# lh3/miniasm

Hardware: AMD Instinct MI355X
Metric: PAF overlaps processed/sec (hit-filter->trans-reduce->GFA) (higher is better)
Workload: dtype u32

## Files before the change

miniasm_amd/csrc/hits.hip:

```cpp
#include "mahip_internal.hpp"

#define COL_QID 0
#define COL_QS 1
#define COL_QE 2
#define COL_TN 3
#define COL_TS 4
#define COL_TE 5
#define COL_ML 6
#define COL_BL 7
#define DEAD 0x80000000u

__global__ __launch_bounds__(256) void k_hit_keys(const ma_hit_t *__restrict__ h, size_t n, uint64_t *__restrict__ key,
                                                   uint32_t *__restrict__ val, uint32_t *__restrict__ keep, unsigned long long *__restrict__ ctr,
                                                   uint32_t q_beg, uint32_t q_end, int bi, int full)
{
	uint32_t cnt = 0;
	for (size_t i = (size_t)blockIdx.x * 256 + threadIdx.x; i < n; i += (size_t)gridDim.x * 256) {
		uint64_t k = h[i].qns;
		uint32_t q = (uint32_t)(k >> 32);
		int in = q >= q_beg && q < q_end;
		cnt += in;
		if (full) key[i] = k, val[i] = (uint32_t)i;
		else key[i] = (uint64_t)q << bi | i;
		if (keep) keep[i] = in;
// ... 244 lines not shown
		else if (i0 < n) q0 = (uint32_t)(skey[i0] >> bi);
		if (q0 > n_seq) q0 = n_seq;
		if (q1 > n_seq) q1 = n_seq;
		uint32_t qprev = __shfl_up(q1, 1, 64);
		if ((threadIdx.x & 63) == 0 && i0 && i0 <= n) qprev = (uint32_t)(skey[i0 - 1] >> bi);
		if (i0 <= n) {
			const uint32_t lo = i0 ? qprev + 1 : q_lo, hi = q0 < q_hi ? q0 : q_hi;
			for (uint32_t r = lo > q_lo ? lo : q_lo; r <= hi; ++r) goff[r] = (uint32_t)i0;
		}
		if (i0 + 1 <= n) { const uint32_t hi = q1 < q_hi ? q1 : q_hi; for (uint32_t r = q0 + 1 > q_lo ? q0 + 1 : q_lo; r <= hi; ++r) goff[r] = (uint32_t)(i0 + 1); }
	}
}

#define SUB_BLOCKS (2u * MA_STREAM_BLOCKS)
static uint32_t sub_chunk(uint32_t R) { uint64_t waves = 4ull * grid_for(R, 4, SUB_BLOCKS), k = waves ? R / waves : 1; return (uint32_t)(k < 1 ? 1 : k > 16 ? 16 : k); }
#define EV_PAD 0xffffffffu
#define SUB_REG_MAX_HITS 512u
#define SUB_CHUNK 16u
#define SUB_LDS_EVENTS 8192u


struct SubFuse {
	const uint2 *cut_sub;
	int min_span, max_hang, min_ovlp;
	uint8_t *r_live;
};
struct SubAcc { uint32_t n_cut, n_flt; uint64_t dp; };

__device__ __forceinline__ uint32_t sub_len(uint2 s) { return s.y - (s.x & 0x7fffffffu); }
__device__ __forceinline__ bool subs_live(uint2 rq, uint2 rt) { return !(rq.x & DEAD) && !(rt.x & DEAD); }

__device__ __forceinline__ int hit_cut(uint2 rq, uint2 rt, uint32_t &qs, uint32_t &qe, uint32_t &ts, uint32_t &te, uint32_t ml, int min_span)
{
	return subs_live(rq, rt) && mc_cut(&qs, &qe, &ts, &te, ml >> 31, (int32_t)rq.x, rq.y, (int32_t)rt.x, rt.y, min_span);
}
__device__ __forceinline__ void store_cut_cols(const HitCols &c, size_t i, uint32_t qs, uint32_t qe, uint32_t ts, uint32_t te, uint32_t oqs, uint32_t oqe, uint32_t ots, uint32_t ote)
{
	if (qs != oqs) c.qs[i] = qs;
	if (qe != oqe) c.qe[i] = qe;
	if (ts != ots) c.ts[i] = ts;
	if (te != ote) c.te[i] = te;
}
__device__ __forceinline__ int hit_flt(uint32_t q, uint32_t qs, uint32_t qe, uint32_t tn, uint32_t ts, uint32_t te, uint32_t ml, uint2 sq, uint2 st,
                                       int max_hang, int min_ovlp, uint64_t &dp, uint8_t *r_live)
{
	mc_arc_t a;
	const uint32_t ql = sub_len(sq), tl = sub_len(st);
	const int r = mc_hit2arc(q, qs, qe, tn, ts, te, ml >> 31, (int)ql, (int)tl, max_hang, .5f, min_ovlp, &a);
	if (r >= 0 || r == MC_HT_QCONT || r == MC_HT_TCONT) {
		dp += r >= 0 ? (uint32_t)r : r == MC_HT_QCONT ? ql : tl;
		r_live[q] = 1;
		return 1;
	}
	return 0;
}
__device__ __forceinline__ void hit_contained_flags(uint32_t q, uint32_t qs, uint32_t qe, uint32_t t, uint32_t ts, uint32_t te, uint32_t ml, uint2 sq, uint2 st,
                                                    int max_hang, float int_frac, int min_ovlp, uint8_t *r_cont, uint8_t *r_used)
{
	mc_arc_t a;
	const int r = mc_hit2arc(q, qs, qe, t, ts, te, ml >> 31, (int)sub_len(sq), (int)sub_len(st), max_hang, int_frac, min_ovlp, &a);
	if (r == MC_HT_QCONT) r_cont[q] = 1;
	else if (r == MC_HT_TCONT) r_cont[t] = 1;
	r_used[q] = 1; r_used[t] = 1;
}

__device__ __forceinline__ int fuse_cut_flt_v(const HitCols &c, uint32_t i, const SubFuse &f, uint32_t q, uint2 rq, uint32_t tn,
                                              uint32_t &qs, uint32_t &qe, uint32_t ml, uint32_t bl, SubAcc &acc, uint2 rt, uint32_t ts, uint32_t te)
{
	int keep = 0;
	const uint32_t oqs = qs, oqe = qe, ots = ts, ote = te;
	if (hit_cut(rq, rt, qs, qe, ts, te, ml, f.min_span)) {
		++acc.n_cut;
		if (hit_flt(q, qs, qe, tn, ts, te, ml, rq, rt, f.max_hang, f.min_ovlp, acc.dp, f.r_live)) {
			keep = 1; ++acc.n_flt;
			store_cut_cols(c, i, qs, qe, ts, te, oqs, oqe, ots, ote);
		}
	}
	if (!keep) c.bl[i] = bl | DEAD;
	return keep;
}
__device__ __forceinline__ int fuse_cut_flt(const HitCols &c, uint32_t i, const SubFuse &f, uint32_t q, uint2 rq, uint32_t tn,
                                            uint32_t &qs, uint32_t &qe, uint32_t ml, uint32_t bl, SubAcc &acc)
{
	return fuse_cut_flt_v(c, i, f, q, rq, tn, qs, qe, ml, bl, acc, f.cut_sub[tn], c.ts[i], c.te[i]);
}

struct SubPre { uint32_t beg, end; uint32_t bl[2], ml[2], qs[2], qe[2], tn[2], ts[2], te[2]; uint2 rt[2], rq; };

template <bool FUSE>
__device__ __forceinline__ void sub_preload(const HitCols &c, const uint32_t *__restrict__ goff, uint32_t q, unsigned lane, SubPre &p)
{
	p.beg = goff[q]; p.end = goff[q + 1];
	const uint32_t H = p.end - p.beg;
#pragma unroll
	for (int h = 0; h < 2; ++h) {
		const uint32_t i = p.beg + h * 64 + lane;
		p.bl[h] = DEAD; p.ml[h] = p.qs[h] = p.qe[h] = p.tn[h] = p.ts[h] = p.te[h] = 0;
		if (H <= 128u && i < p.end) {
			p.bl[h] = c.bl[i]; p.ml[h] = c.ml[i]; p.qs[h] = c.qs[i]; p.qe[h] = c.qe[i]; p.tn[h] = c.tn[i];
			if (FUSE) { p.ts[h] = c.ts[i]; p.te[h] = c.te[i]; }
		}
	}
}

struct SubGather { const uint32_t *pos; uint32_t pstride, pmask; const ma_hit_t *aos; uint32_t *sidx; uint32_t n, chunk, q_lo; };
struct GBounds { uint32_t beg, end; };
struct GKeys { uint32_t beg, end, j[2]; };
struct GRecs { uint32_t beg, end, j[2]; uint4 a[2], b[2]; };

__device__ __forceinline__ uint32_t gather_pos(const SubGather &g, size_t i)
{
	return g.pos[i * g.pstride] & g.pmask;
}
__device__ __forceinline__ void gather_bounds(const uint32_t *__restrict__ goff, uint64_t q, uint32_t n_seq, GBounds &b)
{
	const uint32_t qc = q < n_seq ? (uint32_t)q : n_seq - 1;
	b.beg = goff[qc]; b.end = goff[qc + 1];
}
__device__ __forceinline__ void gather_keys(const SubGather &g, const GBounds &b, unsigned lane, GKeys &k)
{
	k.beg = b.beg; k.end = b.end;
#pragma unroll
	for (int h = 0; h < 2; ++h) {
		const uint32_t i = b.beg + h * 64 + lane, ic = i < g.n ? i : g.n - 1;
		k.j[h] = g.pos[(size_t)ic * g.pstride];
	}
}
__device__ __forceinline__ void gather_recs(const SubGather &g, const GKeys &k, unsigned lane, GRecs &r)
{
	r.beg = k.beg; r.end = k.end;
	const bool mine = k.end - k.beg <= 128u;
	const uint32_t mask = g.pmask;
#pragma unroll
	for (int h = 0; h < 2; ++h) {
		const uint32_t i = k.beg + h * 64 + lane;
		r.j[h] = (mine && i < k.end) ? (k.j[h] & mask) : 0u;
		const uint4 *p = (const uint4*)(g.aos + r.j[h]);
		r.a[h] = p[0]; r.b[h] = p[1];
	}
}
template <int GATHER>
__device__ __forceinline__ void gather_store(const HitCols &c, const SubGather &g, uint32_t i, uint32_t j, uint4 a, uint4 b)
{
	c.qid[i] = a.y; c.qs[i] = a.x; c.qe[i] = a.z; c.tn[i] = a.w;
	c.ts[i] = b.x; c.te[i] = b.y; c.ml[i] = b.z; c.bl[i] = b.w & ~DEAD;
	if (GATHER == 1) g.sidx[i] = j;
}

template <int ITEMS, bool FUSE, int GATHER = 0>
__device__ __forceinline__ uint32_t sub_group_regs(const HitCols &c, uint32_t q, uint32_t beg, uint32_t end, int min_dp, float min_iden,
                                                   int end_clip, uint2 *__restrict__ sub, unsigned lane, const SubFuse &f, SubAcc &acc, const SubPre *pre = nullptr,
                                                   const SubGather *g = nullptr)
{
	uint32_t x[ITEMS];
	int live_any = 0, ev_any = 0;
	uint2 rq = make_uint2(0, 0);
	if (FUSE) rq = pre ? pre->rq : f.cut_sub[q];
	if (GATHER && !pre) {
		constexpr int HB = 4;
#pragma unroll
		for (int h0 = 0; h0 < ITEMS / 2; h0 += HB) {
			uint32_t jj[HB];
			uint4 aa[HB], bb[HB];
#pragma unroll
			for (int k = 0; k < HB; ++k) { const uint32_t i = beg + (h0 + k) * 64 + lane; jj[k] = (h0 + k < ITEMS / 2 && i < end) ? gather_pos(*g, i) : 0u; }
#pragma unroll
			for (int k = 0; k < HB; ++k) { const uint4 *p = (const uint4*)(g->aos + jj[k]); aa[k] = p[0]; bb[k] = p[1]; }
#pragma unroll
			for (int k = 0; k < HB; ++k) {
				const int h = h0 + k;
				const uint32_t i = beg + h * 64 + lane;
				if (h < ITEMS / 2) {
					x[2 * h] = x[2 * h + 1] = EV_PAD;
					if (i < end) {
						uint32_t es, ee;
						gather_store<GATHER>(c, *g, i, jj[k], aa[k], bb[k]);
						live_any = 1;
						if (mc_sub_ok(q, aa[k].x, aa[k].z, aa[k].w, (int32_t)(bb[k].z & 0x7fffffffu), (int32_t)(bb[k].w & ~DEAD), min_iden, end_clip, &es, &ee)) x[2 * h] = es, x[2 * h + 1] = ee, ev_any = 1;
					}
				}
			}
		}
	} else
#pragma unroll
	for (int h = 0; h < ITEMS / 2; ++h) {
		uint32_t i = beg + h * 64 + lane;
		x[2 * h] = x[2 * h + 1] = EV_PAD;
		if (i < end) {
			uint32_t bl, ml, qs, qe, tn, es, ee;
			int alive;
			if (pre) {
				bl = pre->bl[h]; ml = pre->ml[h]; qs = pre->qs[h]; qe = pre->qe[h]; tn = pre->tn[h];
				alive = !(bl & DEAD) && (!FUSE || fuse_cut_flt_v(c, i, f, q, rq, tn, qs, qe, ml, bl, acc, pre->rt[h], pre->ts[h], pre->te[h]));
			} else {
				bl = c.bl[i]; ml = c.ml[i]; qs = c.qs[i]; qe = c.qe[i]; tn = c.tn[i];
				alive = !(bl & DEAD) && (!FUSE || fuse_cut_flt(c, i, f, q, rq, tn, qs, qe, ml, bl, acc));
			}
			if (alive) {
				live_any = 1;
				if (mc_sub_ok(q, qs, qe, tn, (int32_t)(ml & 0x7fffffffu), (int32_t)bl, min_iden, end_clip, &es, &ee)) x[2 * h] = es, x[2 * h + 1] = ee, ev_any = 1;
			}
		}
	}
	if (wv_ballot(live_any) == 0) { if (lane == 0) sub[q] = make_uint2(0, 0); return 0; }
	if (wv_ballot(ev_any) == 0) { if (lane == 0) sub[q] = make_uint2(DEAD, 0); return 0; }
	wave_sort_regs<ITEMS>(x, lane);
	int net = 0;
#pragma unroll
	for (int r = 0; r < ITEMS; ++r) if (x[r] != EV_PAD) net += (x[r] & 1) ? -1 : 1;
	int dp = wv_scan_incl_i32(net, lane) - net;
	const uint32_t NONE = 0xffffffffu;
	uint32_t cur_up = NONE, last_up = NONE, pend_pos = NONE, pend_idx = 0, best_s = 0;
	uint64_t best = 0;
#pragma unroll
	for (int r = 0; r < ITEMS; ++r) {
		uint32_t e = x[r];
		if (e == EV_PAD) continue;
		int old = dp;
		dp += (e & 1) ? -1 : 1;
		if (old < min_dp && dp >= min_dp) cur_up = last_up = e >> 1;
		else if (old >= min_dp && dp < min_dp) {
			if (cur_up != NONE) {
				uint64_t cand = (uint64_t)((e >> 1) - cur_up) << 32 | (0xffffffffu - (lane * ITEMS + r));
				if (cand > best) best = cand, best_s = cur_up;
				cur_up = NONE;
			} else pend_pos = e >> 1, pend_idx = lane * ITEMS + r;
		}
	}
	const uint32_t carry = wv_scan_last_u32(last_up, NONE, lane);
	const uint32_t before = wv_prev_lane_u32(carry, NONE, lane);
	if (pend_pos != NONE && before != NONE) {
		uint64_t cand = (uint64_t)(pend_pos - before) << 32 | (0xffffffffu - pend_idx);
		if (cand > best) best = cand, best_s = before;
	}
	uint64_t gbest = wv_max_u64_full(best);
	uint32_t len = (uint32_t)(gbest >> 32);
	if (len == 0) { if (lane == 0) sub[q] = make_uint2(DEAD, 0); return 0; }
	uint64_t own = wv_ballot(best == gbest);
	uint32_t s = wv_read_lane_u32(best_s, __ffsll((long long)own) - 1);
	if (lane == 0) sub[q] = make_uint2((s - (uint32_t)end_clip) & 0x7fffffffu, s + len + (uint32_t)end_clip);
	return 1;
}

__device__ __forceinline__ unsigned sub_block_id()
{
	const unsigned b = blockIdx.x, g8 = gridDim.x & ~7u;
	return b < g8 ? (b & 7u) * (g8 >> 3) + (b >> 3) : b;
}
#if defined(__HIP__) && defined(__clang__)
#define SUB_WPE_ATTR(F, C, G) __attribute__((amdgpu_waves_per_eu(sub_wpe(F, C, G))))
#else
#define SUB_WPE_ATTR(F, C, G)
#endif
#ifndef SUB_WPE_G0
#define SUB_WPE_G0 7
#endif
#ifndef SUB_WPE_F0
#define SUB_WPE_F0 6
#endif
constexpr unsigned sub_wpe(bool fuse, int cls, int gather) { return gather && cls == 0 ? SUB_WPE_G0 : fuse && cls == 1 ? 5 : fuse && cls == 0 ? SUB_WPE_F0 : 0; }
template <bool FUSE>
__device__ __forceinline__ void sub_flush_acc(unsigned long long *ctr, const SubAcc &acc)
{
	if (FUSE) { blk_add_u64(&ctr[CT_CUT], acc.n_cut); blk_add_u64(&ctr[CT_LIVE], acc.n_flt); blk_add_u64(&ctr[CT_TOTDP], acc.dp); }
}

template <bool FUSE, int CLS, int GATHER = 0>
__global__ __launch_bounds__(256) SUB_WPE_ATTR(FUSE, CLS, GATHER) void k_hit_sub(HitCols c, const uint32_t *__restrict__ goff, uint32_t n_seq,
                                                  int min_dp, float min_iden, int end_clip, uint2 *__restrict__ sub,
                                                  uint32_t *__restrict__ ovf, unsigned long long *__restrict__ ctr, SubFuse f, SubGather g)
{
	const unsigned lane = threadIdx.x & 63, wave = threadIdx.x >> 6;
	uint32_t n_kept = 0;
	SubAcc acc = {0, 0, 0};
	const uint32_t chunk = g.chunk ? g.chunk : 1u;
	if (CLS == 0 && GATHER) {
		const uint64_t stride = (uint64_t)gridDim.x * 4;
		uint64_t q = (uint64_t)g.q_lo + sub_block_id() * 4 + wave;
		GBounds bn;
		GKeys kn;
		GRecs cur, nxt;
		gather_bounds(goff, q, n_seq, bn); gather_keys(g, bn, lane, kn); gather_recs(g, kn, lane, cur);
		gather_bounds(goff, q + stride, n_seq, bn); gather_keys(g, bn, lane, kn);
		gather_bounds(goff, q + 2 * stride, n_seq, bn);
		while (q < n_seq) {
			const uint32_t beg = cur.beg, end = cur.end, H = end - beg;
#pragma unroll
			for (int h = 0; h < 2; ++h) {
				const uint32_t i = beg + h * 64 + lane;
				gather_store<GATHER>(c, g, (H <= 128u && i < end) ? i : g.n + lane, cur.j[h], cur.a[h], cur.b[h]);
			}
			__builtin_amdgcn_sched_barrier(0);
			gather_recs(g, kn, lane, nxt);
			gather_keys(g, bn, lane, kn);
			gather_bounds(goff, q + 3 * stride, n_seq, bn);
			__builtin_amdgcn_sched_barrier(0);
			if (H == 0) { if (lane == 0) sub[q] = make_uint2(0, 0); }
			else if (H <= 128) {
				SubPre pre;
				pre.beg = beg; pre.end = end;
#pragma unroll
				for (int h = 0; h < 2; ++h) {
					pre.bl[h] = cur.b[h].w & ~DEAD; pre.ml[h] = cur.b[h].z; pre.qs[h] = cur.a[h].x; pre.qe[h] = cur.a[h].z; pre.tn[h] = cur.a[h].w;
					pre.ts[h] = pre.te[h] = 0;
				}
				if (H <= 64) n_kept += sub_group_regs<2, false>(c, (uint32_t)q, beg, end, min_dp, min_iden, end_clip, sub, lane, f, acc, &pre);
				else n_kept += sub_group_regs<4, false>(c, (uint32_t)q, beg, end, min_dp, min_iden, end_clip, sub, lane, f, acc, &pre);
			}
			cur = nxt; q += stride;
		}
	} else
	if (CLS == 0) {
		const uint32_t stride = gridDim.x * 4;
		uint32_t q = g.q_lo + sub_block_id() * 4 + wave;
		SubPre cur, nxt;
		if (q < n_seq) sub_preload<FUSE>(c, goff, q, lane, cur);
		while (q < n_seq) {
			const uint32_t qn = q + stride;
			if (FUSE) {
				cur.rq = f.cut_sub[q];
#pragma unroll
				for (int h = 0; h < 2; ++h) cur.rt[h] = (cur.bl[h] & DEAD) ? make_uint2(DEAD, 0) : f.cut_sub[cur.tn[h]];
			}
			if (qn < n_seq) sub_preload<FUSE>(c, goff, qn, lane, nxt);
			const uint32_t beg = cur.beg, end = cur.end, H = end - beg;
			if (H == 0) { if (lane == 0) sub[q] = make_uint2(0, 0); }
			else if (H <= 64) n_kept += sub_group_regs<2, FUSE>(c, q, beg, end, min_dp, min_iden, end_clip, sub, lane, f, acc, &cur);
			else if (H <= 128) n_kept += sub_group_regs<4, FUSE>(c, q, beg, end, min_dp, min_iden, end_clip, sub, lane, f, acc, &cur);
			cur = nxt; q = qn;
		}
	} else
	for (uint64_t qb = (uint64_t)g.q_lo + (uint64_t)(sub_block_id() * 4 + wave) * chunk; qb < n_seq; qb += (uint64_t)gridDim.x * 4 * chunk) {
	const bool in = lane < chunk && qb + lane < n_seq;
	const uint32_t beg_l = in ? goff[qb + lane] : 0, end_l = in ? goff[qb + lane + 1] : 0, H_l = end_l - beg_l;
	unsigned long long todo = wv_ballot(CLS == 1 ? (H_l > 128 && H_l <= 256) : H_l > 256);
	while (todo) {
		const int qbit = __ffsll((long long)todo) - 1;
		todo &= todo - 1;
		const uint32_t q = (uint32_t)qb + (uint32_t)qbit;
		const uint32_t beg = __shfl(beg_l, qbit, 64), end = __shfl(end_l, qbit, 64), H = end - beg;
		if (CLS == 1) {
			if (H > 128 && H <= 256) n_kept += sub_group_regs<8, FUSE, GATHER>(c, q, beg, end, min_dp, min_iden, end_clip, sub, lane, f, acc, nullptr, &g);
		} else {
			if (H > 256 && H <= SUB_REG_MAX_HITS) n_kept += sub_group_regs<16, FUSE, GATHER>(c, q, beg, end, min_dp, min_iden, end_clip, sub, lane, f, acc, nullptr, &g);
			else if (H > SUB_REG_MAX_HITS) {
				if (GATHER)
					for (uint32_t i = beg + lane; i < end; i += 64) {
						const uint32_t j = gather_pos(g, i);
						const uint4 *p = (const uint4*)(g.aos + j);
						gather_store<GATHER>(c, g, i, j, p[0], p[1]);
					}
				if (lane == 0) { unsigned long long k = atomicAdd(&ctr[CT_OVF], 1ull); ovf[k] = q; }
			}
		}
	}
	}
	blk_add_u64(&ctr[CT_REMAIN], lane == 0 ? n_kept : 0);
	sub_flush_acc<FUSE>(ctr, acc);
}

__device__ __forceinline__ uint64_t sub_sweep(const uint32_t *ev, uint32_t *up, uint32_t nev, int min_dp, unsigned lane)
{
	const uint64_t lt = wv_lt(lane), le = wv_le(lane);
	int carry = 0;
	uint32_t nup = 0, ndown = 0;
	uint64_t best = 0;
	for (uint32_t base = 0; base < nev; base += 64) {
		uint32_t i = base + lane;
		int valid = i < nev;
		uint32_t e = valid ? ev[i] : 0;
		int is_end = e & 1;
		uint64_t ms = wv_ballot(valid && !is_end), me = wv_ballot(valid && is_end);
		int dp = carry + __popcll(ms & le) - __popcll(me & le);
		int old = dp - (is_end ? -1 : 1);
		int isup = valid && old < min_dp && dp >= min_dp;
		int isdn = valid && old >= min_dp && dp < min_dp;
		uint64_t mu = wv_ballot(isup), md = wv_ballot(isdn);
		uint32_t ur = nup + __popcll(mu & lt), dr = ndown + __popcll(md & lt);
		if (isup) up[ur] = e >> 1;
		wv_sync();
		if (isdn) {
			uint32_t len = (e >> 1) - up[dr];
			uint64_t cand = (uint64_t)len << 32 | (0xffffffffu - dr);
			best = cand > best ? cand : best;
		}
		carry += __popcll(ms) - __popcll(me);
		nup += __popcll(mu), ndown += __popcll(md);
		wv_sync();
	}
	return wv_max_u64(best);
}

template <bool FUSE>
// ... 1262 lines not shown
```

miniasm_amd/csrc/mahip_internal.hpp:

```cpp
#pragma once
#include <hip/hip_runtime.h>
#include <stdint.h>
#include <stdio.h>
#include <stdlib.h>
#include <string.h>
#include <time.h>
#include <vector>
#include <mutex>
#include <string>
#include "mahip.h"
#include "ma_core.h"

void mahip_set_error(const char *fmt, ...);
extern "C" int ma_timing_level(void);

#define HIPCHK(expr) do { hipError_t e_ = (expr); if (e_ != hipSuccess) { \
	mahip_set_error("%s:%d: %s -> %s", __FILE__, __LINE__, #expr, hipGetErrorString(e_)); return -1; } } while (0)
#define CHK(expr) do { int r_ = (expr); if (r_ != 0) return r_; } while (0)

struct DevBuf {
	void *p = nullptr;
	size_t cap = 0;
	bool ext = false;
};
// ... 89 lines not shown
	void *xfer = nullptr;
	mahip_xfer_info_t xfer_last = {};
	void *paf = nullptr;
	bool paf_keep_odd = false;
	mahip_bgzf_info_t bgzf_last = {};
	mahip_gzip_info_t gzip_last = {};
	mahip_gzip_item_t *gzip_rows = nullptr;
	uint64_t gzip_n_rows = 0;

	hipEvent_t mark_ev[64] = {};
	hipStream_t sub_side[2] = {}; hipEvent_t sub_ev[3] = {};
	uint64_t scan_forms[3] = {0, 0, 0};
	mahip_sort_info_t sort_last = {};
	struct { int n_pass, bits[16], shift[16]; uint32_t fixed7; int groups; } rs_last = {};
	uint64_t tr_inner = 0;
	bool arcs_clean = false;
	bool radix_arcs = false;
	bool sub_fork_failed = false;
	unsigned long long mark_set = 0;
	bool prof = false;
	std::vector<ProfEvent> pev;
	std::vector<size_t> pstack;
	std::vector<ProfAcc> pacc;
};

int dev_reserve(mahip_ctx *c, DevBuf &b, size_t bytes);
void dev_free(mahip_ctx *c, DevBuf &b);
void prof_begin(mahip_ctx *c, const char *name, double alg_bytes);
void prof_end(mahip_ctx *c);
int prof_collect(mahip_ctx *c);
void prof_patch_last(mahip_ctx *c, const char *name, double alg_bytes);

struct ProfScope {
	mahip_ctx *c;
	ProfScope(mahip_ctx *c_, const char *name, double alg_bytes) : c(c_) { if (c->prof) prof_begin(c, name, alg_bytes); }
	~ProfScope() { if (c->prof) prof_end(c); }
};

struct TieLaps {
	mahip_ctx *c; bool on; double t0 = 0;
	static double now() { struct timespec ts; clock_gettime(CLOCK_MONOTONIC, &ts); return ts.tv_sec + ts.tv_nsec * 1e-9; }
	explicit TieLaps(mahip_ctx *c_) : c(c_) { on = ma_timing_level() >= 2; if (on) { (void)hipStreamSynchronize(c->st); t0 = now(); } }
	void lap(const char *what) { if (!on) return; (void)hipStreamSynchronize(c->st); const double t1 = now(); fprintf(stderr, "[T::ties]   %-34s %9.3f ms\n", what, (t1 - t0) * 1e3); t0 = t1; }
};

template <typename T> static inline T *P(DevBuf &b) { return (T*)b.p; }

static inline bool xchg_needs_sync(const mahip_ctx *c) { return c->own_stream && !c->comm; }

enum { CT_LIVE = 0, CT_REMAIN, CT_TOTDP, CT_TOTLEN, CT_OVF, CT_NRED, CT_NMULTI, CT_NASYMM, CT_NSHORT, CT_MAXQID, CT_MAXQS, CT_TOTAL, CT_OVF2, CT_MAXLEN, CT_CUT, CT_TRINNER , CT_PROBED , CT_N };
static_assert(CT_N <= 48, "a named counter would overlap the sticky counters");
enum { CT_STICKY = 48, ST_ARC_TIE_GROUPS = 48, ST_ARC_TIE_ARCS, ST_PUSH_CONFLICTS, ST_HIT_TIES, ST_PUSH_SEEN };
enum { CT_WORDS = 64, CT_XCHG = 64, CT_XCHG_WORDS = 32, CT_ALLOC_WORDS = CT_XCHG + CT_XCHG_WORDS };
int ctr_zero(mahip_ctx *c);
int ctr_fetch(mahip_ctx *c);

int scan_exclusive_u32(mahip_ctx *c, const uint32_t *in, uint32_t *out, size_t n, uint32_t *d_total);
#ifndef RS_MAXBITS
#define RS_MAXBITS 9
#endif
int radix_sort_pairs(mahip_ctx *c, size_t n, int lo0, int hi0, int lo1, int hi1, int *gen);
struct RadixGroups { uint32_t *start; int lo; uint32_t n_id; };
int radix_sort_keys(mahip_ctx *c, size_t n, int lo, int hi, int *gen, bool first_hist_ready = false, const RadixGroups *groups = nullptr);
void radix_first_digit(int lo, int hi, int *shift, int *bits, unsigned *tile);
int radix_reserve_hist(mahip_ctx *c, size_t n);
int radix_group_starts_begin(mahip_ctx *c, uint32_t *start, uint32_t n_id, uint32_t n);
int radix_group_starts_finish(mahip_ctx *c, uint32_t *start, uint32_t n_id);
int scan_chain_begin(mahip_ctx *c, size_t nb, unsigned long long **state, uint32_t **ticket, uint32_t *ticket_base, uint32_t *epoch, size_t n_tickets = 0);
struct WalkWanted { const uint32_t *wcum; uint64_t n_ids; const uint32_t *seg_pos, *seg_len; size_t n_seg; };
int reference_order(mahip_ctx *c, uint64_t *d_keys , size_t n, uint32_t *d_perm, const WalkWanted *w = nullptr);
void walk_scratch_release(mahip_ctx *c);
int hits_reference_rank(mahip_ctx *c, bool collective_ok, bool wanted_only = false);
int hits_qs_bits(mahip_ctx *c);
int hits_need_cols(mahip_ctx *c, const char *who);
int xfer_copy(mahip_ctx *c, void *dev_ptr, void *host_ptr, size_t bytes, int to_device);
void xfer_pool_free(mahip_ctx *c);
int xfer_from_fd(mahip_ctx *c, void *dev_ptr, int fd, size_t bytes);
int xfer_from_fd_at(mahip_ctx *c, void *dev_ptr, int fd, size_t off, size_t bytes);
void paf_free(mahip_ctx *c);
int paf_text_reserve(mahip_ctx *c, size_t nbytes, void **d_text);
void paf_text_loaded(mahip_ctx *c);
int fx_text_reserve(mahip_ctx *c, size_t nbytes, void **d_text);
void fx_text_loaded(mahip_ctx *c);
void clean_free(mahip_ctx *c);
void ug_free(mahip_ctx *c);
void useq_free(mahip_ctx *c);

static inline int bitlen_u64(uint64_t x) { int b = 0; while (x) ++b, x >>= 1; return b; }

static inline unsigned grid_for(size_t n, unsigned per_block, unsigned cap = 0x7fffffffu)
{
	size_t g = (n + per_block - 1) / per_block;
	if (g < 1) g = 1;
	if (g > cap) g = cap;
	return (unsigned)g;
}

#ifdef __HIPCC__
__device__ __forceinline__ unsigned wv_lane() { return __lane_id(); }
__device__ __forceinline__ uint64_t wv_lt(unsigned lane) { return (1ull << lane) - 1ull; }
__device__ __forceinline__ uint64_t wv_le(unsigned lane) { return lane == 63 ? ~0ull : ((1ull << (lane + 1)) - 1ull); }
__device__ __forceinline__ uint64_t wv_ballot(int p) { return __ballot(p); }
__device__ __forceinline__ void wv_sync()
{
	__builtin_amdgcn_fence(__ATOMIC_RELEASE, "workgroup");
	__builtin_amdgcn_wave_barrier();
	__builtin_amdgcn_fence(__ATOMIC_ACQUIRE, "workgroup");
}
__device__ __forceinline__ uint32_t wv_bcast(uint32_t x, int src) { return __shfl(x, src, 64); }
__device__ __forceinline__ uint64_t wv_max_u64(uint64_t x)
{
	for (int o = 32; o > 0; o >>= 1) {
		uint32_t lo = __shfl_xor((uint32_t)x, o, 64), hi = __shfl_xor((uint32_t)(x >> 32), o, 64);
		uint64_t y = (uint64_t)hi << 32 | lo;
		x = y > x ? y : x;
	}
	return x;
}
__device__ __forceinline__ uint32_t wv_sum_u32(uint32_t x)
{
	for (int o = 32; o > 0; o >>= 1) x += __shfl_xor(x, o, 64);
	return x;
}
__device__ __forceinline__ uint64_t wv_sum_u64(uint64_t x)
{
	for (int o = 32; o > 0; o >>= 1) {
		uint32_t lo = __shfl_xor((uint32_t)x, o, 64), hi = __shfl_xor((uint32_t)(x >> 32), o, 64);
		x += (uint64_t)hi << 32 | lo;
	}
	return x;
}
#define WV_DPP(old, x, ctrl, rm) __builtin_amdgcn_update_dpp((int)(old), (int)(x), (ctrl), (rm), 0xf, false)
__device__ __forceinline__ int wv_scan_incl_i32(int x, unsigned lane)
{
	(void)lane;
	x += WV_DPP(0, x, 0x111, 0xf); x += WV_DPP(0, x, 0x112, 0xf); x += WV_DPP(0, x, 0x114, 0xf); x += WV_DPP(0, x, 0x118, 0xf);
	x += WV_DPP(0, x, 0x142, 0xa);
	x += WV_DPP(0, x, 0x143, 0xc);
	return x;
}
__device__ __forceinline__ uint32_t wv_scan_last_u32(uint32_t x, uint32_t none, unsigned lane)
{
	(void)lane;
	uint32_t t;
	t = (uint32_t)WV_DPP(none, x, 0x111, 0xf); x = x == none ? t : x;
	t = (uint32_t)WV_DPP(none, x, 0x112, 0xf); x = x == none ? t : x;
	t = (uint32_t)WV_DPP(none, x, 0x114, 0xf); x = x == none ? t : x;
	t = (uint32_t)WV_DPP(none, x, 0x118, 0xf); x = x == none ? t : x;
	t = (uint32_t)WV_DPP(none, x, 0x142, 0xa); x = x == none ? t : x;
	t = (uint32_t)WV_DPP(none, x, 0x143, 0xc); x = x == none ? t : x;
	return x;
}
__device__ __forceinline__ uint32_t wv_prev_lane_u32(uint32_t x, uint32_t fill, unsigned lane) { (void)lane; return (uint32_t)WV_DPP(fill, x, 0x138, 0xf); }
#define WV_MAX64_STEP(ctrl, rm) do { \
		const uint32_t lo_ = (uint32_t)__builtin_amdgcn_update_dpp(0, (int)(uint32_t)x, (ctrl), (rm), 0xf, false); \
		const uint32_t hi_ = (uint32_t)__builtin_amdgcn_update_dpp(0, (int)(uint32_t)(x >> 32), (ctrl), (rm), 0xf, false); \
		const uint64_t y_ = (uint64_t)hi_ << 32 | lo_; \
		x = y_ > x ? y_ : x; } while (0)
__device__ __forceinline__ uint64_t wv_max_u64_full(uint64_t x)
{
	WV_MAX64_STEP(0x111, 0xf); WV_MAX64_STEP(0x112, 0xf); WV_MAX64_STEP(0x114, 0xf); WV_MAX64_STEP(0x118, 0xf);
	WV_MAX64_STEP(0x142, 0xa); WV_MAX64_STEP(0x143, 0xc);
	return (uint64_t)(uint32_t)__builtin_amdgcn_readlane((int)(uint32_t)(x >> 32), 63) << 32 | (uint32_t)__builtin_amdgcn_readlane((int)(uint32_t)x, 63);
}
#undef WV_MAX64_STEP
__device__ __forceinline__ uint32_t wv_read_lane_u32(uint32_t x, int src) { return (uint32_t)__builtin_amdgcn_readlane((int)x, src); }
#undef WV_DPP
__device__ __forceinline__ void wv_count_add(unsigned long long *ctr, int p)
{
	uint64_t m = __ballot(p);
	if (m && wv_lane() == (unsigned)(__ffsll((long long)m) - 1)) atomicAdd(ctr, (unsigned long long)__popcll(m));
}
__device__ __forceinline__ void blk_add_u64(unsigned long long *ctr, uint64_t x)
{
	__shared__ unsigned long long s_part[8];
	x = wv_sum_u64(x);
	if ((threadIdx.x & 63) == 0) s_part[threadIdx.x >> 6] = x;
	__syncthreads();
	if (threadIdx.x == 0) {
		unsigned long long t = 0;
		for (unsigned w = 0; w < (blockDim.x + 63) / 64; ++w) t += s_part[w];
		if (t) atomicAdd(ctr, t);
	}
	__syncthreads();
}
__device__ __forceinline__ void blk_max_u64(unsigned long long *ctr, uint64_t x)
{
	__shared__ unsigned long long s_part[8];
	x = wv_max_u64(x);
	if ((threadIdx.x & 63) == 0) s_part[threadIdx.x >> 6] = x;
	__syncthreads();
	if (threadIdx.x == 0) {
		unsigned long long t = 0;
		for (unsigned w = 0; w < (blockDim.x + 63) / 64; ++w) t = s_part[w] > t ? s_part[w] : t;
		if (t) atomicMax(ctr, t);
	}
	__syncthreads();
}
__device__ __forceinline__ uint32_t block_excl_scan_256(uint32_t x, uint32_t *s_wave, uint32_t *total)
{
	unsigned lane = threadIdx.x & 63, wave = threadIdx.x >> 6;
	const uint32_t incl = (uint32_t)wv_scan_incl_i32((int)x, lane);
	if (lane == 63) s_wave[wave] = incl;
	__syncthreads();
	uint32_t base = 0, tot = 0;
	for (unsigned w = 0; w < 4; ++w) {
		uint32_t v = s_wave[w];
		if (w < wave) base += v;
		tot += v;
	}
	__syncthreads();
	*total = tot;
	return base + incl - x;
}
#define SC_AGG 1ull
#define SC_INCL 2ull
__device__ __forceinline__ unsigned long long sc_pack(uint32_t epoch, unsigned long long st, uint32_t v) { return (unsigned long long)epoch << 34 | st << 32 | v; }
#define SC_PUBLISH(p, v) __hip_atomic_store((p), (v), __ATOMIC_RELAXED, __HIP_MEMORY_SCOPE_AGENT)
#define SC_PEEK(p) __hip_atomic_load((p), __ATOMIC_RELAXED, __HIP_MEMORY_SCOPE_AGENT)

__device__ __forceinline__ uint32_t sc_look_back(const unsigned long long *state, uint32_t tile, uint32_t epoch, unsigned lane)
{
	uint32_t prefix = 0;
	for (long look = (long)tile - 1;; look -= 64) {
		const long idx = look - (long)lane;
		unsigned long long w = sc_pack(epoch, SC_INCL, 0);
		if (idx >= 0) do { w = SC_PEEK(&state[idx]); } while ((uint32_t)(w >> 34) != epoch || ((w >> 32) & 3ull) == 0);
		const unsigned long long incl = wv_ballot(((w >> 32) & 3ull) == SC_INCL);
		const int first = incl ? __ffsll((long long)incl) - 1 : 63;
		prefix += wv_sum_u32(lane <= (unsigned)first ? (uint32_t)w : 0u);
		if (incl) break;
	}
	return prefix;
}
#define MA_CE(a, b) do { uint32_t lo_ = (a) < (b) ? (a) : (b), hi_ = (a) < (b) ? (b) : (a); (a) = lo_; (b) = hi_; } while (0)

__device__ __forceinline__ uint32_t ma_med3_u32(uint32_t a, uint32_t b, uint32_t c)
{
#if defined(__HIP_DEVICE_COMPILE__)
	uint32_t r;
	asm("v_med3_u32 %0, %1, %2, %3" : "=v"(r) : "v"(a), "v"(b), "v"(c));
	return r;
#else
	const uint32_t lo = a < b ? a : b, hi = a < b ? b : a;
	return c < lo ? lo : c > hi ? hi : c;
#endif
}
#define MA_KEEP(x, y, lower) ma_med3_u32((x), (y), (lower) ? 0u : 0xffffffffu)
__device__ __forceinline__ uint32_t lane_xor(uint32_t x, int m)
{
	const int v = (int)x;
	switch (m) {
	case 1: return (uint32_t)__builtin_amdgcn_mov_dpp(v, 0xB1, 0xf, 0xf, true);
	case 2: return (uint32_t)__builtin_amdgcn_mov_dpp(v, 0x4E, 0xf, 0xf, true);
	case 3: return (uint32_t)__builtin_amdgcn_mov_dpp(v, 0x1B, 0xf, 0xf, true);
	case 7: return (uint32_t)__builtin_amdgcn_mov_dpp(v, 0x141, 0xf, 0xf, true);
	case 15: return (uint32_t)__builtin_amdgcn_mov_dpp(v, 0x140, 0xf, 0xf, true);
	case 8: return (uint32_t)__builtin_amdgcn_mov_dpp(v, 0x128, 0xf, 0xf, true);
	case 4: {
		int t = __builtin_amdgcn_mov_dpp(v, 0x104, 0xf, 0x5, true);
		return (uint32_t)__builtin_amdgcn_update_dpp(t, v, 0x114, 0xf, 0xa, false);
	}
	default: return __shfl_xor(x, m, 64);
	}
}

template <int ITEMS>
__device__ __forceinline__ void wave_sort_regs(uint32_t (&x)[ITEMS], unsigned lane)
{
#pragma unroll
	for (int k = 2; k <= ITEMS; k <<= 1) {
#pragma unroll
		for (int r = 0; r < ITEMS; ++r) { int p = r ^ (k - 1); if (p > r) MA_CE(x[r], x[p]); }
#pragma unroll
		for (int j = k >> 2; j > 0; j >>= 1)
#pragma unroll
			for (int r = 0; r < ITEMS; ++r) if ((r & j) == 0) MA_CE(x[r], x[r | j]);
	}
#pragma unroll
	for (int L = 2; L <= 64; L <<= 1) {
		{
			const bool lower = (lane & (L >> 1)) == 0;
			uint32_t y[ITEMS];
#pragma unroll
			for (int r = 0; r < ITEMS; ++r) y[r] = lane_xor(x[ITEMS - 1 - r], L - 1);
#pragma unroll
			for (int r = 0; r < ITEMS; ++r) x[r] = MA_KEEP(x[r], y[r], lower);
		}
#pragma unroll
		for (int m = L >> 2; m > 0; m >>= 1) {
			const bool lower = (lane & m) == 0;
#pragma unroll
			for (int r = 0; r < ITEMS; ++r) {
				uint32_t y = lane_xor(x[r], m);
				x[r] = MA_KEEP(x[r], y, lower);
			}
		}
#pragma unroll
		for (int j = ITEMS >> 1; j > 0; j >>= 1)
#pragma unroll
			for (int r = 0; r < ITEMS; ++r) if ((r & j) == 0) MA_CE(x[r], x[r | j]);
	}
}

#define MA_STREAM_BLOCKS 2048u

#define MA_BITONIC(T, a, n, tid, STRIDE, SYNC) do { \
	uint32_t P_ = 1; while (P_ < (uint32_t)(n)) P_ <<= 1; \
	for (uint32_t k_ = 2; k_ <= P_; k_ <<= 1) { \
		{ uint32_t h_ = k_ >> 1; \
		  for (uint32_t t_ = (tid); t_ < (P_ >> 1); t_ += (STRIDE)) { \
			uint32_t lo_ = (t_ / h_) * k_ + (t_ % h_), hi_ = lo_ ^ (k_ - 1); \
			if (hi_ < (uint32_t)(n)) { T x_ = (a)[lo_], y_ = (a)[hi_]; if (y_ < x_) (a)[lo_] = y_, (a)[hi_] = x_; } \
		  } SYNC; } \
		for (uint32_t j_ = k_ >> 2; j_ > 0; j_ >>= 1) { \
		  for (uint32_t t_ = (tid); t_ < (P_ >> 1); t_ += (STRIDE)) { \
			uint32_t lo_ = ((t_ & ~(j_ - 1)) << 1) | (t_ & (j_ - 1)), hi_ = lo_ | j_; \
			if (hi_ < (uint32_t)(n)) { T x_ = (a)[lo_], y_ = (a)[hi_]; if (y_ < x_) (a)[lo_] = y_, (a)[hi_] = x_; } \
		  } SYNC; } \
	} } while (0)
#endif
```

Baseline: 6.584 billion.

## Replace event-sort depth sweep with separate start/end sorts and rank-shift max-depth detection

The sub-region search now sorts interval starts and ends as two separate half-size arrays, instead of sorting a single interleaved event array of twice the size. It then finds regions covered by at least min_dp intervals by comparing the (min_dp-1)-shifted sorted starts against the sorted ends. This drops the per-event depth prefix scan and the pending carry logic, replacing them with a register rotation, a ds_bpermute lane shift and head/tail flags. The intent is cheaper sorting (two width-M sorts in place of one width-2M sort) and a simpler sweep. The risk is tie-breaking and boundary semantics differing from the original event ordering, plus added bpermute traffic.

```diff
diff --git a/miniasm_amd/csrc/hits.hip b/miniasm_amd/csrc/hits.hip
--- a/miniasm_amd/csrc/hits.hip
+++ b/miniasm_amd/csrc/hits.hip
@@ -420,7 +420,8 @@
                                                    int end_clip, uint2 *__restrict__ sub, unsigned lane, const SubFuse &f, SubAcc &acc, const SubPre *pre = nullptr,
                                                    const SubGather *g = nullptr)
 {
-	uint32_t x[ITEMS];
+	constexpr int M = ITEMS / 2;
+	uint32_t s[M], e[M];
 	int live_any = 0, ev_any = 0;
 	uint2 rq = make_uint2(0, 0);
 	if (FUSE) rq = pre ? pre->rq : f.cut_sub[q];
@@ -439,12 +440,12 @@
 				const int h = h0 + k;
 				const uint32_t i = beg + h * 64 + lane;
 				if (h < ITEMS / 2) {
-					x[2 * h] = x[2 * h + 1] = EV_PAD;
+					s[h] = e[h] = EV_PAD;
 					if (i < end) {
 						uint32_t es, ee;
 						gather_store<GATHER>(c, *g, i, jj[k], aa[k], bb[k]);
 						live_any = 1;
-						if (mc_sub_ok(q, aa[k].x, aa[k].z, aa[k].w, (int32_t)(bb[k].z & 0x7fffffffu), (int32_t)(bb[k].w & ~DEAD), min_iden, end_clip, &es, &ee)) x[2 * h] = es, x[2 * h + 1] = ee, ev_any = 1;
+						if (mc_sub_ok(q, aa[k].x, aa[k].z, aa[k].w, (int32_t)(bb[k].z & 0x7fffffffu), (int32_t)(bb[k].w & ~DEAD), min_iden, end_clip, &es, &ee)) s[h] = es >> 1, e[h] = ee >> 1, ev_any = 1;
 					}
 				}
 			}
@@ -453,7 +454,7 @@
 #pragma unroll
 	for (int h = 0; h < ITEMS / 2; ++h) {
 		uint32_t i = beg + h * 64 + lane;
-		x[2 * h] = x[2 * h + 1] = EV_PAD;
+		s[h] = e[h] = EV_PAD;
 		if (i < end) {
 			uint32_t bl, ml, qs, qe, tn, es, ee;
 			int alive;
@@ -466,47 +467,59 @@
 			}
 			if (alive) {
 				live_any = 1;
-				if (mc_sub_ok(q, qs, qe, tn, (int32_t)(ml & 0x7fffffffu), (int32_t)bl, min_iden, end_clip, &es, &ee)) x[2 * h] = es, x[2 * h + 1] = ee, ev_any = 1;
+				if (mc_sub_ok(q, qs, qe, tn, (int32_t)(ml & 0x7fffffffu), (int32_t)bl, min_iden, end_clip, &es, &ee)) s[h] = es >> 1, e[h] = ee >> 1, ev_any = 1;
 			}
 		}
 	}
 	if (wv_ballot(live_any) == 0) { if (lane == 0) sub[q] = make_uint2(0, 0); return 0; }
 	if (wv_ballot(ev_any) == 0) { if (lane == 0) sub[q] = make_uint2(DEAD, 0); return 0; }
-	wave_sort_regs<ITEMS>(x, lane);
-	int net = 0;
-#pragma unroll
-	for (int r = 0; r < ITEMS; ++r) if (x[r] != EV_PAD) net += (x[r] & 1) ? -1 : 1;
-	int dp = wv_scan_incl_i32(net, lane) - net;
+	if (min_dp < 1) { if (lane == 0) sub[q] = make_uint2(DEAD, 0); return 0; }
+	wave_sort2_regs<M>(s, e, lane);
+	const uint32_t d = (uint32_t)(min_dp - 1) < 64u * M ? (uint32_t)(min_dp - 1) : 64u * M, dl = d / M, dr = d % M;
+	uint32_t A[M], B[M];
+#pragma unroll
+	for (int r = 0; r < M; ++r) A[r] = s[r];
+#pragma unroll
+	for (int b = 1; b < M; b <<= 1)
+		if (dr & b) {
+			uint32_t t[M];
+#pragma unroll
+			for (int r = 0; r < M; ++r) t[r] = A[(r + b) % M];
+#pragma unroll
+			for (int r = 0; r < M; ++r) A[r] = t[r];
+		}
+#pragma unroll
+	for (int r = 0; r < M; ++r) A[r] = wv_lane_up_u32(A[r], dl + (r + dr >= (uint32_t)M ? 1u : 0u), EV_PAD, lane);
+#pragma unroll
+	for (int r = 0; r + 1 < M; ++r) B[r] = A[r + 1];
+	B[M - 1] = wv_next_lane_u32(A[0], EV_PAD, lane);
+	bool head[M], tail[M];
+	{
+		bool lprev = wv_prev_lane_u32(B[M - 1] <= e[M - 1] ? 1u : 0u, 0u, lane) != 0;
+#pragma unroll
+		for (int r = 0; r < M; ++r) {
+			const bool val = A[r] <= e[r], lnk = B[r] <= e[r];
+			head[r] = val && !lprev; tail[r] = val && !lnk;
+			lprev = lnk;
+		}
+	}
 	const uint32_t NONE = 0xffffffffu;
-	uint32_t cur_up = NONE, last_up = NONE, pend_pos = NONE, pend_idx = 0, best_s = 0;
-	uint64_t best = 0;
-#pragma unroll
-	for (int r = 0; r < ITEMS; ++r) {
-		uint32_t e = x[r];
-		if (e == EV_PAD) continue;
-		int old = dp;
-		dp += (e & 1) ? -1 : 1;
-		if (old < min_dp && dp >= min_dp) cur_up = last_up = e >> 1;
-		else if (old >= min_dp && dp < min_dp) {
-			if (cur_up != NONE) {
-				uint64_t cand = (uint64_t)((e >> 1) - cur_up) << 32 | (0xffffffffu - (lane * ITEMS + r));
-				if (cand > best) best = cand, best_s = cur_up;
-				cur_up = NONE;
-			} else pend_pos = e >> 1, pend_idx = lane * ITEMS + r;
-		}
-	}
-	const uint32_t carry = wv_scan_last_u32(last_up, NONE, lane);
-	const uint32_t before = wv_prev_lane_u32(carry, NONE, lane);
-	if (pend_pos != NONE && before != NONE) {
-		uint64_t cand = (uint64_t)(pend_pos - before) << 32 | (0xffffffffu - pend_idx);
-		if (cand > best) best = cand, best_s = before;
-	}
-	uint64_t gbest = wv_max_u64_full(best);
-	uint32_t len = (uint32_t)(gbest >> 32);
+	uint32_t last = NONE;
+#pragma unroll
+	for (int r = 0; r < M; ++r) if (head[r]) last = A[r];
+	uint32_t cur = wv_prev_lane_u32(wv_scan_last_u32(last, NONE, lane), NONE, lane);
+	uint32_t best_len = 0, best_s = 0;
+#pragma unroll
+	for (int r = 0; r < M; ++r) {
+		if (head[r]) cur = A[r];
+		const uint32_t len = e[r] - cur;
+		if (tail[r] && len > best_len) best_len = len, best_s = cur;
+	}
+	const uint64_t gbest = wv_max_u64_full((uint64_t)best_len << 32 | (63u - lane));
+	const uint32_t len = (uint32_t)(gbest >> 32);
 	if (len == 0) { if (lane == 0) sub[q] = make_uint2(DEAD, 0); return 0; }
-	uint64_t own = wv_ballot(best == gbest);
-	uint32_t s = wv_read_lane_u32(best_s, __ffsll((long long)own) - 1);
-	if (lane == 0) sub[q] = make_uint2((s - (uint32_t)end_clip) & 0x7fffffffu, s + len + (uint32_t)end_clip);
+	const uint32_t st = wv_read_lane_u32(best_s, 63 - (int)(uint32_t)gbest);
+	if (lane == 0) sub[q] = make_uint2((st - (uint32_t)end_clip) & 0x7fffffffu, st + len + (uint32_t)end_clip);
 	return 1;
 }
 
diff --git a/miniasm_amd/csrc/mahip_internal.hpp b/miniasm_amd/csrc/mahip_internal.hpp
--- a/miniasm_amd/csrc/mahip_internal.hpp
+++ b/miniasm_amd/csrc/mahip_internal.hpp
@@ -265,6 +265,12 @@
 	return x;
 }
 __device__ __forceinline__ uint32_t wv_prev_lane_u32(uint32_t x, uint32_t fill, unsigned lane) { (void)lane; return (uint32_t)WV_DPP(fill, x, 0x138, 0xf); }
+__device__ __forceinline__ uint32_t wv_next_lane_u32(uint32_t x, uint32_t fill, unsigned lane) { (void)lane; return (uint32_t)WV_DPP(fill, x, 0x130, 0xf); }
+__device__ __forceinline__ uint32_t wv_lane_up_u32(uint32_t x, uint32_t up, uint32_t fill, unsigned lane)
+{
+	const uint32_t v = (uint32_t)__builtin_amdgcn_ds_bpermute((int)(((lane + up) & 63u) << 2), (int)x);
+	return lane + up < 64u ? v : fill;
+}
 #define WV_MAX64_STEP(ctrl, rm) do { \
 		const uint32_t lo_ = (uint32_t)__builtin_amdgcn_update_dpp(0, (int)(uint32_t)x, (ctrl), (rm), 0xf, false); \
 		const uint32_t hi_ = (uint32_t)__builtin_amdgcn_update_dpp(0, (int)(uint32_t)(x >> 32), (ctrl), (rm), 0xf, false); \
@@ -413,6 +419,44 @@
 		for (int j = ITEMS >> 1; j > 0; j >>= 1)
 #pragma unroll
 			for (int r = 0; r < ITEMS; ++r) if ((r & j) == 0) MA_CE(x[r], x[r | j]);
+	}
+}
+
+template <int M>
+__device__ __forceinline__ void wave_sort2_regs(uint32_t (&a)[M], uint32_t (&b)[M], unsigned lane)
+{
+#pragma unroll
+	for (int k = 2; k <= M; k <<= 1) {
+#pragma unroll
+		for (int r = 0; r < M; ++r) { int p = r ^ (k - 1); if (p > r) { MA_CE(a[r], a[p]); MA_CE(b[r], b[p]); } }
+#pragma unroll
+		for (int j = k >> 2; j > 0; j >>= 1)
+#pragma unroll
+			for (int r = 0; r < M; ++r) if ((r & j) == 0) { MA_CE(a[r], a[r | j]); MA_CE(b[r], b[r | j]); }
+	}
+#pragma unroll
+	for (int L = 2; L <= 64; L <<= 1) {
+		{
+			const bool lower = (lane & (L >> 1)) == 0;
+			uint32_t ya[M], yb[M];
+#pragma unroll
+			for (int r = 0; r < M; ++r) { ya[r] = lane_xor(a[M - 1 - r], L - 1); yb[r] = lane_xor(b[M - 1 - r], L - 1); }
+#pragma unroll
+			for (int r = 0; r < M; ++r) { a[r] = MA_KEEP(a[r], ya[r], lower); b[r] = MA_KEEP(b[r], yb[r], lower); }
+		}
+#pragma unroll
+		for (int m = L >> 2; m > 0; m >>= 1) {
+			const bool lower = (lane & m) == 0;
+#pragma unroll
+			for (int r = 0; r < M; ++r) {
+				const uint32_t ya = lane_xor(a[r], m), yb = lane_xor(b[r], m);
+				a[r] = MA_KEEP(a[r], ya, lower); b[r] = MA_KEEP(b[r], yb, lower);
+			}
+		}
+#pragma unroll
+		for (int j = M >> 1; j > 0; j >>= 1)
+#pragma unroll
+			for (int r = 0; r < M; ++r) if ((r & j) == 0) { MA_CE(a[r], a[r | j]); MA_CE(b[r], b[r | j]); }
 	}
 }
 
```

Result: slower. 6.472 billion (-1.7%).
